# cielavenir/7bgzf

Measured on NVIDIA B200. Metric: BGZF compress GB/s (uncompressed), higher is better.
Workload: dtype u8

## Files before the change

7bgzf_b200/csrc/bgzf_block.h:

```cpp
#ifndef BGZF_BLOCK_H
#define BGZF_BLOCK_H

#include <stdint.h>
#include <stdio.h>

#if defined(__CUDACC__)
#define BG_HD __host__ __device__ __forceinline__
#else
#define BG_HD static inline
#endif
#if defined(BG_CHECK) && defined(__CUDA_ARCH__)
#define BG_ASSERT(cond) do { if (!(cond)) { printf("BG_ASSERT failed: %s (%s:%d) block %d thread %d\n", #cond, __FILE__, __LINE__, (int)blockIdx.x, (int)threadIdx.x); __trap(); } } while (0)
#else
#define BG_ASSERT(cond) do { } while (0)
#endif


#define BG_MAX_BLOCK 65536u
#define BG_DATA_BYTES (BG_MAX_BLOCK + 32u)
#define BG_HASH_BITS 14
#define BG_HASH_SIZE (1u << BG_HASH_BITS)
#define BG_NOPOS 0xFFFFu
#define BG_CHUNK 68u
#define BG_THREADS 1024u
// ... 81 lines not shown
    const uint32_t *crcpow;
    const uint16_t *perm;
    uint32_t n;
    uint32_t frame;
    BgParams prm;
};

BG_HD uint32_t bg_frame(uint32_t hdr, uint32_t trl, uint32_t final, uint32_t piece, uint32_t hist = 0) { return hdr | (trl << 8) | (final << 16) | (piece << 17) | ((hist / BG_CHUNK) << 18); }
BG_HD uint32_t bg_f_hist(const BgCtx &c) { return (c.frame >> 18) * BG_CHUNK; }
BG_HD uint32_t bg_f_hdr(const BgCtx &c) { return c.frame & 0xffu; }
BG_HD uint32_t bg_f_trl(const BgCtx &c) { return (c.frame >> 8) & 0xffu; }
BG_HD uint32_t bg_f_final(const BgCtx &c) { return (c.frame >> 16) & 1u; }
BG_HD bool bg_f_piece(const BgCtx &c) { return (c.frame >> 17) & 1u; }


BG_HD uint32_t bg_ld32(const uint32_t *w, uint32_t p)
{
    uint32_t i = p >> 2, s = (p & 3u) * 8u;
    uint32_t lo = w[i], hi = w[i + 1];
#if defined(__CUDA_ARCH__)
    return __funnelshift_r(lo, hi, p << 3);
#else
    return s ? (lo >> s) | (hi << (32u - s)) : lo;
#endif
}

BG_HD uint32_t bg_ld8(const uint32_t *w, uint32_t p) { return ((const uint8_t *)w)[p]; }

BG_HD uint32_t bg_funnel(uint32_t lo, uint32_t hi, uint32_t s)
{
#if defined(__CUDA_ARCH__)
    return __funnelshift_r(lo, hi, s);
#else
    return s ? (lo >> s) | (hi << (32u - s)) : lo;
#endif
}

BG_HD int bg_bsr(uint32_t v)
{
#if defined(__CUDA_ARCH__)
    return 31 - __clz(v);
#else
    return 31 - __builtin_clz(v);
#endif
}

BG_HD int bg_ctz(uint32_t v)
{
#if defined(__CUDA_ARCH__)
    return __ffs(v) - 1;
#else
    return __builtin_ctz(v);
#endif
}

BG_HD uint32_t bg_brev(uint32_t v, int nbits)
{
#if defined(__CUDA_ARCH__)
    return __brev(v) >> (32 - nbits);
#else
    uint32_t r = 0;
    for (int i = 0; i < nbits; i++)
        r |= ((v >> i) & 1u) << (nbits - 1 - i);
    return r;
#endif
}

BG_HD void bg_add32(uint32_t *a, uint32_t v)
{
#if defined(__CUDA_ARCH__)
    atomicAdd(a, v);
#else
    *a += v;
#endif
}

BG_HD uint32_t bg_fetch_add32(uint32_t *a, uint32_t v)
{
#if defined(__CUDA_ARCH__)
    return atomicAdd(a, v);
#else
    uint32_t old = *a;
    *a += v;
    return old;
#endif
}

BG_HD void bg_or32(uint32_t *a, uint32_t v)
{
#if defined(__CUDA_ARCH__)
    atomicOr(a, v);
#else
    *a |= v;
#endif
}

BG_HD uint32_t bg_len_slot(uint32_t len, uint32_t *nextra, uint32_t *extra)
{
    uint32_t l = len - 3;
    if (l < 8) { *nextra = 0; *extra = 0; return l; }
    if (len == 258) { *nextra = 0; *extra = 0; return 28; }
    uint32_t nb = (uint32_t)bg_bsr(l) - 2;
    *nextra = nb;
    *extra = l & ((1u << nb) - 1);
    return 8 + 4 * (nb - 1) + ((l >> nb) & 3);
}

BG_HD uint32_t bg_off_slot(uint32_t off, uint32_t *nextra, uint32_t *extra)
{
    uint32_t d = off - 1;
    if (d < 4) { *nextra = 0; *extra = 0; return d; }
    uint32_t b = (uint32_t)bg_bsr(d);
    *nextra = b - 1;
    *extra = d & ((1u << (b - 1)) - 1);
    return 2 * b + ((d >> (b - 1)) & 1);
}

BG_HD uint32_t bg_len_slot_extra_bits(uint32_t slot) { return slot < 8 || slot == 28 ? 0 : (slot - 4) >> 2; }
BG_HD uint32_t bg_off_slot_extra_bits(uint32_t slot) { return slot < 4 ? 0 : (slot - 2) >> 1; }

BG_HD uint32_t bg_static_llen(uint32_t sym) { return sym < 144 ? 8 : sym < 256 ? 9 : sym < 280 ? 7 : 8; }


#define BG_CRC_POLY 0xEDB88320u

BG_HD uint32_t bg_crc_mul(uint32_t a, uint32_t b)
{
    uint32_t p = 0;
    for (int i = 0; i < 32; i++) {
        p ^= b & (0u - ((a >> (31 - i)) & 1u));
        b = (b >> 1) ^ (BG_CRC_POLY & (0u - (b & 1u)));
    }
    return p;
}

BG_HD uint32_t bg_crc_byte(const uint32_t *tab, uint32_t r, uint32_t b) { return tab[(r ^ b) & 0xff] ^ (r >> 8); }

BG_HD uint32_t bg_mw(uint32_t len, uint32_t off) { return (len << 16) | (0xffffu - off); }
BG_HD uint32_t bg_mw_off(uint32_t r) { return 0xffffu - (r & 0xffffu); }


BG_HD void bg_phase_init(const BgCtx &c, uint32_t t, uint32_t T)
{
    for (uint32_t i = t; i < BG_HASH_SIZE; i += T)
        c.head[i] = BG_NOPOS;
    if (t < 256)
        c.litflag[t] = 0;
    if (t < 28)
        ((uint8_t *)c.dataw)[c.n + t] = 0;
    if (t < BG_S_COUNT)
        c.scal[t] = 0;
}

BG_HD void bg_phase_scan(const BgCtx &c, uint32_t t, uint32_t T)
{
    const uint32_t n = c.n;
    for (uint32_t p = t; p < n; p += T)
        c.litflag[bg_ld8(c.dataw, p)] = 1;
    const uint32_t hw = bg_f_hist(c) >> 2;
    const uint32_t m = (n >> 2) - hw;
    const uint32_t k = T - 1 - t;
    const uint32_t endw = m >= BG_CRC_WORDS * k ? m - BG_CRC_WORDS * k : 0;
    const uint32_t begw = endw >= BG_CRC_WORDS ? endw - BG_CRC_WORDS : 0;
    uint32_t r = 0;
    if (endw > begw) {
        r = begw == 0 ? 0xFFFFFFFFu : 0u;
        for (uint32_t w = begw; w < endw; w++) {
            uint32_t v = c.dataw[hw + w];
            r = bg_crc_byte(c.crctab, r, v & 0xff);
            r = bg_crc_byte(c.crctab, r, (v >> 8) & 0xff);
            r = bg_crc_byte(c.crctab, r, (v >> 16) & 0xff);
            r = bg_crc_byte(c.crctab, r, v >> 24);
        }
        r = bg_crc_mul(r, c.crcpow[k]);
    }
#if defined(__CUDA_ARCH__)
    for (int d = 16; d > 0; d >>= 1)
        r ^= __shfl_xor_sync(0xffffffffu, r, d);
    if ((t & 31u) == 0 && r)
        atomicXor(&c.scal[BG_S_CRC], r);
#else
    c.scal[BG_S_CRC] ^= r;
#endif
}

BG_HD void bg_phase_count(const BgCtx &c, uint32_t t, uint32_t T)
{
    (void)T;
    if (t < 256 && c.litflag[t])
        bg_add32(&c.scal[BG_S_NUSED], 1);
}

BG_HD uint32_t bg_min_match_len(uint32_t nused, int depth, uint32_t n)
{
    uint32_t ml;
    if (n < 512) return 3;
    ml = nused < 6 ? 9 : nused < 8 ? 8 : nused < 10 ? 7 : nused < 16 ? 6 : nused < 45 ? 5 : nused < 80 ? 4 : 3;
    if (depth < 16) {
        uint32_t cap = depth < 5 ? 4 : depth < 10 ? 5 : 7;
        if (ml > cap) ml = cap;
    }
    return ml;
}

BG_HD void bg_phase_settle(const BgCtx &c, uint32_t t, uint32_t T)
{
    (void)T;
    if (t != 0) return;
    const uint32_t n = c.n;
    uint32_t r = c.scal[BG_S_CRC];
    if (((n - bg_f_hist(c)) >> 2) == 0) r = 0xFFFFFFFFu;
    for (uint32_t p = n & ~3u; p < n; p++)
        r = bg_crc_byte(c.crctab, r, bg_ld8(c.dataw, p));
    c.scal[BG_S_CRC] = ~r;
    c.scal[BG_S_MINLEN] = bg_min_match_len(c.scal[BG_S_NUSED], c.prm.depth, n);
    c.scal[BG_S_DEPTH] = c.scal[BG_S_NUSED] >= 80 && c.prm.opt_passes == 0 ? (uint32_t)c.prm.depth + ((uint32_t)c.prm.depth + 1) / 2 : (uint32_t)c.prm.depth;
    c.scal[BG_S_HBYTES] = bg_min_match_len(c.scal[BG_S_NUSED], 1000, n) >= 5 ? (uint32_t)c.prm.hlong : 4u;
    if (c.scal[BG_S_MINLEN] == 3 && c.prm.depth >= 8) c.scal[BG_S_HBYTES] = 3;
}

BG_HD uint32_t bg_hash(const uint32_t *dataw, uint32_t p, uint32_t hbytes)
{
    uint32_t v = bg_ld32(dataw, p);
    if (hbytes == 3) v &= 0xffffffu;
    uint32_t h = v * 0x1E35A7BDu;
    if (hbytes == 5)
        h ^= bg_ld8(dataw, p + 4) * 0x9E3779B1u;
    else if (hbytes == 8)
        h ^= bg_ld32(dataw, p + 4) * 0x9E3779B1u;
    return h >> (32 - BG_HASH_BITS);
}

BG_HD void bg_phase_hash(const BgCtx &c, uint32_t t, uint32_t T)
{
    const uint32_t n = c.n, hb = c.scal[BG_S_HBYTES];
    for (uint32_t p = t; p < n; p += T)
        c.prev[p] = (p + hb <= n) ? (uint16_t)bg_hash(c.dataw, p, hb) : (uint16_t)BG_NOPOS;
}

BG_HD void bg_build_sequential(const BgCtx &c)
{
    for (uint32_t p = 0; p < c.n; p++) {
        uint32_t h = c.prev[p];
        if (h == BG_NOPOS) continue;
        c.prev[p] = c.head[h];
        c.head[h] = (uint16_t)p;
    }
}

BG_HD uint32_t bg_match_len(const uint32_t *dw, uint32_t p, uint32_t q, uint32_t l, uint32_t maxl)
{
    if (l >= maxl) return maxl;
    const uint32_t sp = (p & 3u) * 8u, sq = (q & 3u) * 8u;
    const uint32_t *wp = dw + ((p + l) >> 2), *wq = dw + ((q + l) >> 2);
    uint32_t plo = wp[0], qlo = wq[0];
    for (;;) {
        const uint32_t p1 = wp[1], q1 = wq[1], p2 = wp[2], q2 = wq[2];
        const uint32_t x1 = bg_funnel(plo, p1, sp) ^ bg_funnel(qlo, q1, sq);
        if (x1) { l += (uint32_t)bg_ctz(x1) >> 3; break; }
        const uint32_t x2 = bg_funnel(p1, p2, sp) ^ bg_funnel(q1, q2, sq);
        if (x2) { l += 4u + ((uint32_t)bg_ctz(x2) >> 3); break; }
        l += 8;
        if (l >= maxl) break;
        plo = p2;
        qlo = q2;
        wp += 2;
        wq += 2;
    }
    return l > maxl ? maxl : l;
}

BG_HD bool bg_in_window(uint32_t p, uint32_t q) { return p - q - 1u < 32768u; }


#define BG_B_TODO 0u
#define BG_B_MARK 8192u
#define BG_B_QUEUE 8192u
#define BG_B_RINGR 20480u
#define BG_B_RING 28672u
#define BG_QUEUE_WORDS 96u
#define BG_SCAN_CHUNK 2u
#define BG_QUEUE_WORDS_SHALLOW 160u
#define BG_SCAN_CHUNK_SHALLOW 4u

BG_HD bool bg_match_ok(uint32_t r, uint32_t minlen);

struct BgSearchPrm {
    uint32_t depth, nice, minlen;
    bool h3;
};
BG_HD BgSearchPrm bg_search_prm(const BgCtx &c)
{
    BgSearchPrm s;
    s.depth = c.scal[BG_S_DEPTH];
    s.nice = (uint32_t)c.prm.nice;
    s.minlen = c.scal[BG_S_MINLEN];
    s.h3 = c.scal[BG_S_HBYTES] == 3;
    return s;
}

template <bool H3>
BG_HD uint32_t bg_nearest_t(const BgCtx &c, const BgSearchPrm &sp, uint32_t p, bool *deep, uint32_t *target)
{
    uint32_t maxl = c.n - p;
    if (maxl > 258) maxl = 258;
    *deep = false;
    *target = p + 1;
    if (maxl < (uint32_t)BG_MIN_LOOKUP) return 0;
    const uint32_t q = c.prev[p];
    if (!bg_in_window(p, q)) return 0;
    const uint32_t *dw = c.dataw;
    uint32_t len = 3;
    if (H3) {
        len = 2;
        if (((bg_ld32(dw, q) ^ bg_ld32(dw, p)) & 0xffffffu) == 0) len = bg_match_len(dw, p, q, 0, maxl);
    } else if (bg_ld32(dw, q) == bg_ld32(dw, p)) {
        len = bg_match_len(dw, p, q, 4, maxl);
    }
    *deep = sp.depth > 1 && len < sp.nice && len < maxl && bg_in_window(p, c.prev[q]);
    if (len <= (H3 ? 2u : 3u)) return 0;
    const uint32_t r = bg_mw(len, p - q);
    if (bg_match_ok(r, sp.minlen)) *target = p + len;
    return r;
}
BG_HD uint32_t bg_nearest(const BgCtx &c, const BgSearchPrm &sp, uint32_t p, bool *deep, uint32_t *target)
{
    return sp.h3 ? bg_nearest_t<true>(c, sp, p, deep, target) : bg_nearest_t<false>(c, sp, p, deep, target);
}

BG_HD uint32_t bg_off_bin(uint32_t off) { return off <= 32u ? 0u : off <= 512u ? 1u : off <= 8192u ? 2u : 3u; }

BG_HD void bg_cand_init(const BgCtx &c, uint32_t p, uint32_t r)
{
    uint32_t *cd = c.cand + 4u * p;
    const uint32_t k = r ? bg_off_bin(bg_mw_off(r)) : 4u;
    cd[0] = k == 0 ? r : 0u; cd[1] = k == 1 ? r : 0u; cd[2] = k == 2 ? r : 0u; cd[3] = k == 3 ? r : 0u;
}

BG_HD void bg_phase_search_clear(const BgCtx &c, uint32_t t, uint32_t T)
{
    uint32_t *w = (uint32_t *)(c.regb + BG_B_TODO);
    for (uint32_t i = t; i < (BG_B_MARK + 8256u) / 4u; i += T) w[i] = 0;
}

BG_HD void bg_phase_search1(const BgCtx &c, uint32_t t, uint32_t T)
{
    uint32_t *elig = (uint32_t *)(c.regb + BG_B_TODO), *mark = (uint32_t *)(c.regb + BG_B_MARK);
    const uint32_t hist = bg_f_hist(c);
    if (t == 0) bg_or32(&mark[hist >> 5], 1u << (hist & 31u));
    const BgSearchPrm sp = bg_search_prm(c);
    for (uint32_t p = t; p < c.n; p += T) {
        bool deep;
        uint32_t target;
        if (p < hist) {
            c.R[p] = 0;
            if (c.prm.opt_passes > 0) bg_cand_init(c, p, 0);
            continue;
        }
        c.R[p] = bg_nearest(c, sp, p, &deep, &target);
        if (c.prm.opt_passes > 0) bg_cand_init(c, p, c.R[p]);
        if (deep) bg_or32(&elig[p >> 5], 1u << (p & 31u));
        bg_or32(&mark[target >> 5], 1u << (target & 31u));
    }
}

BG_HD void bg_phase_search_todo(const BgCtx &c, uint32_t t, uint32_t T, uint32_t own, uint32_t parts)
{
    uint32_t *todo = (uint32_t *)(c.regb + BG_B_TODO);
    const uint32_t *mark = (const uint32_t *)(c.regb + BG_B_MARK);
    for (uint32_t i = t; i < 2048u; i += T) {
        const uint32_t m = mark[i], pm = i ? mark[i - 1] : 0u;
// ... 1192 lines not shown
```

7bgzf_b200/csrc/bgzf_compress.cu:

```cuda
#include <cuda_runtime.h>
#include <stdint.h>

#include <atomic>
#include <cstring>

#include "bgzf_block.h"
#include "bgzf_kernels.h"

#define SM_DATA 0u
#define SM_REGA (BG_DATA_BYTES)
#define SM_REGB (SM_REGA + 131072u)
#define SM_CRCTAB (SM_REGB + 32768u)
#define SM_LITFLAG (SM_CRCTAB + 1024u)
#define SM_SCAL (SM_LITFLAG + 256u)
#define SM_MBAR (SM_SCAL + 4u * BG_S_COUNT)
#define SM_FRONTIER (SM_MBAR + 8u)
#define SM_SCAN (SM_MBAR + 16u)
#define SM_READY (SM_SCAN + 4u * 36u)
#define SM_TOTAL (SM_READY + 128u)

extern "C" size_t bgzf_compress_smem_bytes(void) { return SM_TOTAL; }

__device__ __forceinline__ uint32_t smem_u32(const void *p) { return (uint32_t)__cvta_generic_to_shared(p); }

// ... 460 lines not shown
            }
        }
    }
    __syncwarp();
    drain_queue<H3>(c, queue, 0u, cnt, lane);
}

__device__ __forceinline__ uint32_t cluster_rank()
{
    uint32_t r;
    asm volatile("mov.u32 %0, %%cluster_ctarank;" : "=r"(r));
    return r;
}
__device__ __forceinline__ uint32_t cluster_size()
{
    uint32_t r;
    asm volatile("mov.u32 %0, %%cluster_nctarank;" : "=r"(r));
    return r;
}
__device__ __forceinline__ void cluster_sync()
{
    asm volatile("barrier.cluster.arrive.release.aligned;\n\tbarrier.cluster.wait.acquire.aligned;" ::: "memory");
}

__device__ __forceinline__ void dp_segment_warp(const BgCtx &c, uint32_t w, uint32_t lane, uint32_t *ring)
{
    uint32_t a, b, e;
    bg_dp_segment_bounds(c.n, w, 32, &a, &b, &e);
    if (a >= b) return;
    const uint8_t *rb = c.regb;
    const uint4 *cand4 = (const uint4 *)c.cand;
    uint4 *stage = (uint4 *)(c.regb + BG_B_XTAB) + w * 32u;
    if (lane == 0) ring[e & (BG_DP_RING - 1)] = 0;
    const uint4 zero4 = make_uint4(0, 0, 0, 0);
    uint32_t top = e - 1;
    uint4 next = top >= lane && top - lane >= a ? __ldcg(cand4 + (top - lane)) : zero4;
    for (;;) {
        const uint4 mine = next;
        const uint32_t q = top - lane;
        const bool more = top >= a + 32u;
        if (more) next = top - 32u >= lane && top - 32u - lane >= a ? __ldcg(cand4 + (top - 32u - lane)) : zero4;
        {
            uint32_t oc = 0, litc = 0, m0 = 0, m1 = 0, m2 = 0, m3 = 0;
            if (top >= lane && q >= a) {
                const uint32_t cd[4] = { mine.x, mine.y, mine.z, mine.w };
#pragma unroll
                for (int k = 0; k < 4; k++) {
                    uint32_t nbx, exx;
                    if (cd[k]) oc |= (uint32_t)rb[BG_B_OFFCOST + bg_off_slot(bg_mw_off(cd[k]), &nbx, &exx)] << (8 * k);
                }
                m0 = mine.x >> 16;
                m1 = max(m0, mine.y >> 16);
                m2 = max(m1, mine.z >> 16);
                m3 = max(m2, mine.w >> 16);
                litc = rb[BG_B_LITCOST + bg_ld8(c.dataw, q)];
            }
            stage[lane] = make_uint4(m0 | (m1 << 16), m2 | (m3 << 16), oc, litc);
        }
        __syncwarp();
        const uint32_t steps = top - a + 1 < 32u ? top - a + 1 : 32u;
        uint32_t mybest = 0;
        for (uint32_t j = 0; j < steps; j++) {
            const uint32_t p = top - j;
            const uint4 st = stage[j];
            const uint32_t M0 = st.x & 0xffffu, M1 = st.x >> 16, M2 = st.y & 0xffffu, M3 = st.y >> 16;
            uint32_t maxl = e - p;
            if (M3 < maxl) maxl = M3;
            uint32_t best = 0xffffffffu;
            if (lane == 0) best = bg_dp_pack(st.w + ring[(p + 1) & (BG_DP_RING - 1)], 1, 0);
            uint32_t l = 3 + lane;
            if (l <= maxl) {
#pragma unroll 1
                do {
                    const uint32_t k = (l > M0 ? 1u : 0u) + (l > M1 ? 1u : 0u) + (l > M2 ? 1u : 0u);
                    const uint32_t oc = (st.z >> (8 * k)) & 0xffu;
                    const uint32_t v = bg_dp_pack(rb[BG_B_LENCOST + l] + oc + ring[(p + l) & (BG_DP_RING - 1)], l, k);
                    best = v < best ? v : best;
                    l += 32;
                } while (l <= maxl);
            }
            best = __reduce_min_sync(0xffffffffu, best);
            if (lane == j) {
                ring[p & (BG_DP_RING - 1)] = best >> 11;
                mybest = best;
            }
            __syncwarp();
        }
        if (lane < steps && q < b) {
            const uint32_t l = (mybest >> 2) & 511u, k = mybest & 3u;
            if (l == 1) {
                c.stepcode[q] = 0;
            } else {
                const uint32_t off = bg_mw_off(k == 0 ? mine.x : k == 1 ? mine.y : k == 2 ? mine.z : mine.w);
                c.stepcode[q] = (uint8_t)(l <= 256 ? l - 2 : 255);
                c.R[q] = bg_mw(l, off);
            }
        }
        if (!more) break;
        top -= 32u;
    }
}

__device__ __forceinline__ uint32_t chunk_class(const BgCtx &c, uint32_t ch)
{
    if (ch * BG_CHUNK >= c.n) return 0u;
    const uint32_t *sc = (const uint32_t *)(c.stepcode + ch * BG_CHUNK);
    uint32_t zeros = 0;
#pragma unroll
    for (uint32_t k = 0; k < BG_CHUNK / 4u; k++) {
        const uint32_t v = sc[k];
        zeros += __popc((v - 0x01010101u) & ~v & 0x80808080u);
    }
    return zeros >= 64u ? 7u : zeros >> 3;
}

__device__ __forceinline__ void chunk_order_count(const BgCtx &c, uint32_t t, uint32_t &cls, uint32_t &rank)
{
    const uint32_t lane = t & 31u, warp = t >> 5;
    uint32_t *cnt = (uint32_t *)(c.regb + BG_B_CLASSCNT);
    cls = chunk_class(c, t);
    rank = 0;
#pragma unroll
    for (uint32_t k = 0; k < 8u; k++) {
        const unsigned m = __ballot_sync(0xffffffffu, cls == k);
        if (cls == k) rank = __popc(m & ((1u << lane) - 1u));
        if (lane == k) cnt[k * 32u + warp] = __popc(m);
    }
}

__device__ __forceinline__ void chunk_order_scan(const BgCtx &c, uint32_t t)
{
    if (t >= 32u) return;
    uint32_t *cnt = (uint32_t *)(c.regb + BG_B_CLASSCNT);
    uint32_t v[8], sum = 0;
#pragma unroll
    for (uint32_t k = 0; k < 8u; k++) { v[k] = cnt[t * 8u + k]; sum += v[k]; }
    uint32_t inc = sum;
    for (int d = 1; d < 32; d <<= 1) {
        const uint32_t y = __shfl_up_sync(0xffffffffu, inc, d);
        if (t >= (uint32_t)d) inc += y;
    }
    uint32_t run = inc - sum;
#pragma unroll
    for (uint32_t k = 0; k < 8u; k++) { cnt[t * 8u + k] = run; run += v[k]; }
}

__device__ __forceinline__ void chunk_order_place(const BgCtx &c, uint32_t t, uint32_t cls, uint32_t rank)
{
    const uint32_t *cnt = (const uint32_t *)(c.regb + BG_B_CLASSCNT);
    BG_ASSERT(cls < 8u && cnt[cls * 32u + (t >> 5)] + rank < BG_MAX_CHUNKS);
    ((uint16_t *)(c.regb + BG_B_PERM))[cnt[cls * 32u + (t >> 5)] + rank] = (uint16_t)t;
}

__device__ __forceinline__ void bitonic_sort_512(uint32_t *keys, uint32_t t)
{
    for (uint32_t k = 2; k <= 512; k <<= 1) {
        for (uint32_t j = k >> 1; j > 0; j >>= 1) {
            if (t < 512) {
                uint32_t x = t ^ j;
                if (x > t) {
                    uint32_t a = keys[t], b = keys[x];
                    bool up = (t & k) == 0;
                    if ((a > b) == up) { keys[t] = b; keys[x] = a; }
                }
            }
            __syncthreads();
        }
    }
}

__device__ __forceinline__ uint32_t block_exclusive_scan_1024(uint32_t *v, uint32_t *scratch, uint32_t t)
{
    const uint32_t lane = t & 31u, warp = t >> 5;
    uint32_t x = v[t], inc = x;
    for (int d = 1; d < 32; d <<= 1) {
        uint32_t y = __shfl_up_sync(0xffffffffu, inc, d);
        if (lane >= (uint32_t)d) inc += y;
    }
    if (lane == 31) scratch[warp] = inc;
    __syncthreads();
    if (warp == 0) {
        uint32_t w = scratch[lane], winc = w;
        for (int d = 1; d < 32; d <<= 1) {
            uint32_t y = __shfl_up_sync(0xffffffffu, winc, d);
            if (lane >= (uint32_t)d) winc += y;
        }
        scratch[lane] = winc - w;
        if (lane == 31) scratch[32] = winc;
    }
    __syncthreads();
    v[t] = scratch[warp] + inc - x;
    uint32_t total = scratch[32];
    __syncthreads();
    return total;
}

__device__ __forceinline__ void gather_member(const uint32_t *src, uint32_t n, uint8_t *dst, uint32_t t, uint32_t nthr)
{
    const uint32_t head = (uint32_t)((4u - ((uintptr_t)dst & 3u)) & 3u);
    if (n <= head + 4) {
        for (uint32_t i = t; i < n; i += nthr) dst[i] = (uint8_t)(__ldcg(src + (i >> 2)) >> (8u * (i & 3u)));
        return;
    }
    if (t < head) dst[t] = (uint8_t)(__ldcg(src) >> (8u * t));
    const uint32_t words = (n - head) >> 2;
    uint32_t *dw = (uint32_t *)(dst + head);
    const uint32_t sh = head * 8u;
    for (uint32_t i = t; i < words; i += nthr)
        dw[i] = __funnelshift_r(__ldcg(src + i), __ldcg(src + i + 1), sh);
    const uint32_t done = head + words * 4u;
    if (t < n - done) dst[done + t] = (uint8_t)(__ldcg(src + ((done + t) >> 2)) >> (8u * ((done + t) & 3u)));
}

__device__ __forceinline__ uint32_t block_exclusive_scan_1024(uint32_t *v, uint32_t *scratch, uint32_t t);

__device__ __forceinline__ void fused_compaction(const BgzfCompressArgs &a, uint32_t *v, uint32_t *scratch, uint32_t t)
{
    uint64_t carry = *a.gather_total;
    for (uint32_t start = 0; start < a.nblocks; start += 1024u) {
        const uint32_t i = start + t;
        v[t] = i < a.nblocks ? __ldcg(a.out_len + i) : 0u;
        __syncthreads();
        const uint32_t total = block_exclusive_scan_1024(v, scratch, t);
        if (i < a.nblocks) a.gather_off[i] = carry + v[t];
        carry += total;
        __syncthreads();
    }
    if (t == 0) *a.gather_total = carry;
    __syncthreads();
    const uint32_t grp = t >> 8, gt = t & 255u;
    for (uint32_t b = grp; b < a.nblocks; b += BG_THREADS / 256u) {
        BG_ASSERT(__ldcg(a.out_len + b) <= BG_SLOT_BYTES && a.gather_off[b] + __ldcg(a.out_len + b) <= carry);
        gather_member((const uint32_t *)(a.slots + (size_t)b * BG_SLOT_BYTES), __ldcg(a.out_len + b), a.gather_out + a.gather_off[b], gt, 256u);
    }
}

#define PROF_MARK(i)                                                        \
    do {                                                                    \
        if (prof && t == 0) {                                               \
            long long now_ = clock64();                                     \
            atomicAdd((unsigned long long *)&prof[i], (unsigned long long)(now_ - tprev_)); \
            tprev_ = now_;                                                  \
        }                                                                   \
    } while (0)

template <bool SPLIT>
__device__ __forceinline__ void compress_blocks(BgzfCompressArgs &a)
{
    extern __shared__ __align__(128) uint8_t smem[];
    const uint32_t t = threadIdx.x, T = BG_THREADS;
    uint64_t *mbar = (uint64_t *)(smem + SM_MBAR);
    uint32_t *scan_scratch = (uint32_t *)(smem + SM_SCAN);
    unsigned long long *prof = a.prof;
    long long tprev_ = prof ? clock64() : 0;
    uint32_t *const pscr = scan_scratch;

    BgCtx c;
    c.dataw = (uint32_t *)(smem + SM_DATA);
    c.prev = (uint16_t *)(smem + SM_REGA);
    c.stepcode = smem + SM_REGA;
    c.jump8 = smem + SM_REGA + 65536u;
    c.offarr = (uint16_t *)(smem + SM_REGA + 65536u);
    c.head = (uint16_t *)(smem + SM_REGB);
    c.regb = smem + SM_REGB;
    c.crctab = (uint32_t *)(smem + SM_CRCTAB);
    c.litflag = smem + SM_LITFLAG;
    c.scal = (uint32_t *)(smem + SM_SCAL);
    const uint32_t crank = SPLIT ? cluster_rank() : 0u, csize = SPLIT ? cluster_size() : 1u;
    const uint32_t unit = SPLIT ? blockIdx.x / csize : blockIdx.x;
    uint32_t *const unit_scratch = a.scratch + (size_t)unit * (SPLIT ? BGZF_SCRATCH_WORDS + BGZF_SPLIT_EXTRA_WORDS : BGZF_SCRATCH_WORDS);
    c.R = unit_scratch;
    c.cand = a.cand ? a.cand + (size_t)unit * (4u * BG_MAX_BLOCK) : nullptr;
    c.crcpow = a.crcpow;
    c.prm = a.prm;
    c.frame = bg_frame(a.hdr_bytes ? a.hdr_bytes : 18u, 8u, 1u, 0u);
    c.perm = (const uint16_t *)(smem + SM_REGB + BG_B_PERM);

    if (t < 256) c.crctab[t] = a.crctab[t];
    if (t == 0) {
        mbar_init(mbar, 1);
        asm volatile("fence.mbarrier_init.release.cluster;" ::: "memory");
    }
    __syncthreads();
    uint32_t parity = 0;

    for (uint32_t b = unit; b < a.nblocks; b += SPLIT ? a.nblocks : gridDim.x) {
        const uint8_t *src;
        uint32_t n;
        if (a.in_off) {
            src = a.in + a.in_off[b];
            n = a.in_len[b];
        } else {
            const uint64_t off = (uint64_t)b * a.block_size;
            src = a.in + off;
            const uint64_t rem = a.in_bytes - off;
            n = rem < a.block_size ? (uint32_t)rem : a.block_size;
        }
        c.out = (uint32_t *)(a.slots + (size_t)b * BG_SLOT_BYTES);
        if (a.piece_mode) {
            const uint64_t gb = a.piece_base + b;
            const bool first = gb % a.member_blocks == 0, last = (gb + 1) % a.member_blocks == 0 || gb + 1 == a.piece_total;
            uint32_t hist = 0;
            if (a.history && !first && !a.in_off) {
                const uint64_t in_member = (gb % a.member_blocks) * a.block_size, in_buffer = (uint64_t)a.lead + (uint64_t)b * a.block_size;
                uint64_t h = in_member < in_buffer ? in_member : in_buffer;
                if (h > a.history) h = a.history;
                hist = (uint32_t)h - (uint32_t)h % BG_HISTORY_STEP;
            }
            src -= hist;
            n += hist;
            c.frame = bg_frame(first ? a.head_gap : 0u, last ? a.tail_gap : 0u, last && !a.no_final ? 1u : 0u, 1u, hist);
        }
        c.n = n;

        const bool aligned = (((uintptr_t)src) & 15u) == 0;
        const uint32_t bulk = aligned ? (n & ~15u) : 0u;
        if (bulk) {
            if (t == 0) {
                fence_proxy_async();
                mbar_expect_tx(mbar, bulk);
                tma_load_1d(smem + SM_DATA, src, bulk, mbar);
            }
        }
        for (uint32_t i = bulk + t; i < n; i += T)
            smem[SM_DATA + i] = src[i];
        bg_phase_init(c, t, T);
        if (bulk) {
            mbar_wait(mbar, parity);
            parity ^= 1u;
        }
        __syncthreads();
        PROF_MARK(0);

        bg_phase_scan(c, t, T);
        __syncthreads();
        bg_phase_count(c, t, T);
        __syncthreads();
        bg_phase_settle(c, t, T);
        __syncthreads();
        PROF_MARK(1);
        PROF_MARK(2);
        uint4 *hi = (uint4 *)(c.R + BG_MAX_BLOCK + 32);
        if (SPLIT) {
            uint4 *xprev = (uint4 *)(unit_scratch + BGZF_SCRATCH_WORDS);
            build_peers_phase(c, hi, t & 31u, t >> 5, BG_THREADS / 32u, crank, csize, xprev, nullptr, nullptr, 0);
            cluster_sync();
            import_peer_tiles(c, xprev, t, crank, csize);
            __syncthreads();
            PROF_MARK(3);
            if (t < 32u * BG_LINKERS) build_link_phase(c, hi, t >> 5, t & 31u, &c.scal[BG_S_WLIST], nullptr, nullptr, 0);
        } else {
            volatile uint8_t *ready = (volatile uint8_t *)(smem + SM_READY);
            if (t < 128u) ready[t] = 0;
            if (prof && t == 0) { pscr[0] = 0; pscr[1] = 0; pscr[2] = 0xffffffffu; }
            __syncthreads();
            const long long t0 = prof ? clock64() : 0;
            if (t < 32u * BG_LINKERS) {
                build_link_phase(c, hi, t >> 5, t & 31u, &c.scal[BG_S_WLIST], ready, prof, t0);
            } else {
                build_peers_phase(c, hi, t & 31u, (t >> 5) - BG_LINKERS, BG_THREADS / 32u - BG_LINKERS, 0u, 1u, nullptr, ready, prof, t0);
                if (prof && (t & 31u) == 0) atomicMax(&pscr[0], (uint32_t)(clock64() - t0));
            }
        }
        __syncthreads();
        PROF_MARK(10);
        {
            bg_phase_search_clear(c, t, T);
            if (SPLIT) cluster_sync();
            else __syncthreads();
            const long long t1 = prof ? clock64() : 0;
            search_nearest<SPLIT>(c, t, crank, csize);
            if (!SPLIT && prof && (t & 31u) == 0) {
                const uint32_t d = (uint32_t)(clock64() - t1);
                atomicMax(&pscr[1], d);
                atomicMin(&pscr[2], d);
            }
            if (SPLIT) cluster_sync();
            else __syncthreads();
            if (!SPLIT && prof && t == 0) {
                atomicAdd(&prof[22], (unsigned long long)pscr[0]);
                atomicAdd(&prof[26], (unsigned long long)pscr[1]);
                atomicAdd(&prof[27], (unsigned long long)pscr[2]);
            }
            PROF_MARK(21);
            if (c.scal[BG_S_DEPTH] > 1) {
                bg_phase_search_todo(c, t, T, crank, csize);
                __syncthreads();
                const bool h3 = c.scal[BG_S_HBYTES] == 3;
                if (c.scal[BG_S_DEPTH] <= 24u) {
                    if (h3) search_deep_batches<true>(c, t, crank, csize);
                    else search_deep_batches<false>(c, t, crank, csize);
                } else {
                    if (h3) search_deep<true>(c, t, crank, csize);
                    else search_deep<false>(c, t, crank, csize);
                }
            }
        }
        if (SPLIT) {
            cluster_sync();
            if (crank) return;
        }
        __syncthreads();
        PROF_MARK(4);
        for (int pass = 0; pass <= c.prm.opt_passes; pass++) {
            if (pass == 0) {
                bg_phase_accept(c, t, T);
            } else {
                bg_phase_costs(c, t, T);
                __syncthreads();
                dp_segment_warp(c, t >> 5, t & 31u, (uint32_t *)(smem + SM_REGA + 65536u) + (t >> 5) * BG_DP_RING);
            }
            __syncthreads();
            if (bg_f_hist(c)) {
                bg_phase_history_steps(c, t, T);
                __syncthreads();
            }
            PROF_MARK(15);
            bg_phase_jump(c, t, T);
            __syncthreads();
            PROF_MARK(5);
            bg_phase_walk_clear(c, t, T);
            bg_phase_clear_freq(c, t, T);
            __syncthreads();
            bg_phase_walk_mark(c, t, T);
            __syncthreads();
            bg_phase_walk_list(c, t, T);
            __syncthreads();
            PROF_MARK(16);
            bg_phase_walk_a(c, t, T);
            __syncthreads();
            PROF_MARK(17);
            bg_phase_walk_b(c, t, T);
            uint32_t ccls, crnk;
            chunk_order_count(c, t, ccls, crnk);
            __syncthreads();
            PROF_MARK(18);
            bg_phase_walk_c(c, t, T);
            chunk_order_scan(c, t);
            __syncthreads();
            chunk_order_place(c, t, ccls, crnk);
            __syncthreads();
            PROF_MARK(6);
            bg_phase_tally(c, t, T);
            __syncthreads();
            bg_phase_lkeys(c, t, T);
            __syncthreads();
            PROF_MARK(7);
            bitonic_sort_512((uint32_t *)(c.regb + BG_B_KEYS), t);
            PROF_MARK(11);
            bg_phase_huff_prep(c, t, T);
            __syncthreads();
            bg_phase_huff(c, t, T);
            __syncthreads();
            bg_phase_huff_depth(c, t, T);
            __syncthreads();
            bg_phase_huff_fix(c, t, T);
            __syncthreads();
            bg_phase_huff_assign(c, t, T);
            __syncthreads();
            PROF_MARK(12);
        }
        bg_phase_hdr1(c, t, T);
        __syncthreads();
        bg_phase_hdr2(c, t, T);
        __syncthreads();
        bg_phase_hdr3(c, t, T);
        __syncthreads();
        const uint32_t nitems = block_exclusive_scan_1024((uint32_t *)(c.regb + BG_B_CBITS), scan_scratch, t);
        bg_phase_hdr4(c, t, T);
        __syncthreads();
        bg_phase_hdr4b(c, t, T);
        __syncthreads();
        bg_phase_hdr5(c, t, T, nitems);
        __syncthreads();
        PROF_MARK(13);
        bg_phase_decide_b(c, t, T);
        __syncthreads();
        bg_phase_codes_a(c, t, T);
        __syncthreads();
        bg_phase_codes_b(c, t, T);
        __syncthreads();
        bg_phase_codes_c(c, t, T);
        __syncthreads();
        bg_phase_tabs(c, t, T);
        __syncthreads();
        PROF_MARK(8);
        bg_phase_hdr_bits(c, t, T);
        bg_phase_sizes(c, t, T);
        __syncthreads();
        PROF_MARK(19);
        block_exclusive_scan_1024((uint32_t *)(c.regb + BG_B_CBITS), scan_scratch, t);
        block_exclusive_scan_1024((uint32_t *)(c.regb + BG_B_IOFF), scan_scratch, t);
        PROF_MARK(20);
        bg_phase_zero_out(c, t, T);
        __syncthreads();
        PROF_MARK(14);
        bg_phase_emit(c, t, T);
        if (t == 0) {
            const uint32_t st = c.scal[BG_S_STATUS];
            a.out_len[b] = st ? 0u : bg_f_hdr(c) + c.scal[BG_S_PAYLOAD] + bg_f_trl(c);
            if (a.crc_out) a.crc_out[b] = c.scal[BG_S_CRC];
            a.status[b] = st;
            if (st) atomicOr(a.err_flag, 1u);
        }
        fence_proxy_async();
        __syncthreads();
        PROF_MARK(9);
    }
    if (!SPLIT && a.gather_out) {
        __threadfence();
        __syncthreads();
        if (t == 0) scan_scratch[35] = atomicAdd(a.done_count, 1u) == gridDim.x - 1u ? 1u : 0u;
        __syncthreads();
        if (scan_scratch[35]) {
            __threadfence();
            fused_compaction(a, (uint32_t *)(smem + SM_REGB), scan_scratch, t);
        }
    }
}

__global__ void __launch_bounds__(BG_THREADS, 1)
bgzf_compress_kernel(BgzfCompressArgs a)
{
    compress_blocks<false>(a);
}

__global__ void __launch_bounds__(BG_THREADS, 1)
bgzf_compress_split_kernel(BgzfCompressArgs a)
{
    compress_blocks<true>(a);
}

__global__ void __launch_bounds__(1024, 1)
bgzf_scan_kernel(const uint32_t *len, uint64_t *off, uint32_t nmax, const uint64_t *count_dev, const uint64_t *base_dev,
                 uint64_t *total_out)
{
    __shared__ uint32_t v[1024];
    __shared__ uint32_t scratch[36];
    const uint32_t t = threadIdx.x;
    uint32_t n = nmax;
    if (count_dev) { const uint64_t cd = *count_dev; n = cd < nmax ? (uint32_t)cd : nmax; }
    uint64_t carry = base_dev ? *base_dev : 0ull;
    __syncthreads();
    for (uint32_t start = 0; start < n; start += 1024) {
        const uint32_t i = start + t;
        v[t] = i < n ? len[i] : 0u;
        __syncthreads();
        const uint32_t total = block_exclusive_scan_1024(v, scratch, t);
        if (i < n) off[i] = carry + v[t];
        carry += total;
        __syncthreads();
    }
    if (t == 0) *total_out = carry;
}

__global__ void __launch_bounds__(256)
bgzf_gather_kernel(const uint8_t *slots, const uint32_t *len, const uint64_t *off, uint32_t nblocks, uint8_t *out,
                   const uint64_t *total, int append_eof)
{
    const uint32_t b = blockIdx.x, t = threadIdx.x;
    if (b == nblocks) {
        if (append_eof && t < 28) {
            const uint8_t eof[28] = { 0x1f, 0x8b, 0x08, 0x04, 0, 0, 0, 0, 0, 0xff, 0x06, 0, 0x42, 0x43, 0x02, 0,
                                      0x1b, 0, 0x03, 0, 0, 0, 0, 0, 0, 0, 0, 0 };
            out[*total + t] = eof[t];
        }
        return;
    }
    const uint32_t n = len[b];
    const uint32_t *src = (const uint32_t *)(slots + (size_t)b * BG_SLOT_BYTES);
    uint8_t *dst = out + off[b];
    const uint32_t head = (uint32_t)((4u - ((uintptr_t)dst & 3u)) & 3u);
    if (n <= head + 4) {
        for (uint32_t i = t; i < n; i += blockDim.x) dst[i] = ((const uint8_t *)src)[i];
        return;
    }
    if (t < head) dst[t] = ((const uint8_t *)src)[t];
    const uint32_t words = (n - head) >> 2;
    uint32_t *dw = (uint32_t *)(dst + head);
    const uint32_t sh = head * 8u;
    for (uint32_t i = t; i < words; i += blockDim.x)
        dw[i] = __funnelshift_r(src[i], src[i + 1], sh);
    const uint32_t done = head + words * 4u;
    if (t < n - done) dst[done + t] = ((const uint8_t *)src)[done + t];
}

__global__ void __launch_bounds__(256)
bgzf_deliver_kernel(const uint8_t *slots, const uint32_t *len, const uint64_t *out_off, uint8_t *host_out, uint32_t n)
{
    const uint32_t b = blockIdx.x, t = threadIdx.x;
    if (b >= n) return;
    const uint32_t nbytes = len[b];
    const uint4 *src = (const uint4 *)(slots + (size_t)b * BG_SLOT_BYTES);
    uint4 *dst = (uint4 *)(host_out + out_off[b]);
    for (uint32_t i = t; i < (nbytes + 15u) / 16u; i += blockDim.x) dst[1u + i] = src[i];
    if (t == 0) dst[0] = make_uint4(nbytes, 0u, 0u, 0u);
}

extern "C" cudaError_t bgzf_launch_deliver(const uint8_t *slots, const uint32_t *len, const uint64_t *out_off, uint8_t *host_out, uint32_t n,
                                           cudaStream_t stream)
{
    bgzf_deliver_kernel<<<n, 256, 0, stream>>>(slots, len, out_off, host_out, n);
    return cudaGetLastError();
}

extern "C" cudaError_t bgzf_launch_compress(const BgzfCompressArgs *a, int grid, cudaStream_t stream)
{
    static std::atomic<unsigned long long> configured{0};
    int dev = 0;
    cudaGetDevice(&dev);
    if (!((configured.load() >> dev) & 1ull)) {
        cudaError_t e = cudaFuncSetAttribute(bgzf_compress_kernel, cudaFuncAttributeMaxDynamicSharedMemorySize, (int)SM_TOTAL);
        if (e != cudaSuccess) return e;
        configured.fetch_or(1ull << dev);
    }
    bgzf_compress_kernel<<<grid, BG_THREADS, SM_TOTAL, stream>>>(*a);
    return cudaGetLastError();
}

extern "C" cudaError_t bgzf_launch_compress_split(const BgzfCompressArgs *a, int csize, cudaStream_t stream)
{
    static std::atomic<unsigned long long> configured{0};
    int dev = 0;
    cudaGetDevice(&dev);
    if (!((configured.load() >> dev) & 1ull)) {
        cudaError_t e = cudaFuncSetAttribute(bgzf_compress_split_kernel, cudaFuncAttributeMaxDynamicSharedMemorySize, (int)SM_TOTAL);
// ... 35 lines not shown
```

Measured before the change: 32.99.

## Overlap CRC with Huffman tree build and replace bitonic sort with rank sort

Splits the CRC computation out of the initial scan so that it runs on the idle warps while four warps build the Huffman trees behind a named barrier. The 512-element bitonic sort, with its many block-wide barriers, is replaced by a direct counting rank for the literal/length keys. Distance-tree construction and the precode header are done by single warps. The aim is to cut block-wide synchronisation and serial phases in the per-block pipeline. The cost is more complex warp specialisation, and the CRC now depends on a pass==0 condition in the non-split path.

```diff
diff --git a/7bgzf_b200/csrc/bgzf_block.h b/7bgzf_b200/csrc/bgzf_block.h
--- a/7bgzf_b200/csrc/bgzf_block.h
+++ b/7bgzf_b200/csrc/bgzf_block.h
@@ -257,36 +257,58 @@
         c.scal[t] = 0;
 }
 
+BG_HD void bg_phase_census(const BgCtx &c, uint32_t t, uint32_t T)
+{
+    for (uint32_t p = t; p < c.n; p += T)
+        c.litflag[bg_ld8(c.dataw, p)] = 1;
+}
+
+BG_HD void bg_crc_slices(const BgCtx &c, uint32_t u, uint32_t U)
+{
+    const uint32_t hw = bg_f_hist(c) >> 2;
+    const uint32_t m = (c.n >> 2) - hw;
+    const uint32_t *d = c.dataw + hw;
+    uint32_t acc = 0;
+    for (uint32_t k0 = u; k0 < BG_THREADS; k0 += 2 * U) {
+        const uint32_t k1 = k0 + U;
+        const uint32_t e0 = m >= BG_CRC_WORDS * k0 ? m - BG_CRC_WORDS * k0 : 0;
+        const uint32_t e1 = k1 < BG_THREADS && m >= BG_CRC_WORDS * k1 ? m - BG_CRC_WORDS * k1 : 0;
+        const uint32_t b0 = e0 >= BG_CRC_WORDS ? e0 - BG_CRC_WORDS : 0, b1 = e1 >= BG_CRC_WORDS ? e1 - BG_CRC_WORDS : 0;
+        if (e0 == b0) break;
+        uint32_t r0 = b0 == 0 ? 0xFFFFFFFFu : 0u, r1 = b1 == 0 ? 0xFFFFFFFFu : 0u;
+        for (uint32_t i = 0; i < BG_CRC_WORDS; i++) {
+            if (b0 + i < e0) {
+                const uint32_t v = d[b0 + i];
+                r0 = bg_crc_byte(c.crctab, r0, v & 0xff);
+                r0 = bg_crc_byte(c.crctab, r0, (v >> 8) & 0xff);
+                r0 = bg_crc_byte(c.crctab, r0, (v >> 16) & 0xff);
+                r0 = bg_crc_byte(c.crctab, r0, v >> 24);
+            }
+            if (b1 + i < e1) {
+                const uint32_t v = d[b1 + i];
+                r1 = bg_crc_byte(c.crctab, r1, v & 0xff);
+                r1 = bg_crc_byte(c.crctab, r1, (v >> 8) & 0xff);
+                r1 = bg_crc_byte(c.crctab, r1, (v >> 16) & 0xff);
+                r1 = bg_crc_byte(c.crctab, r1, v >> 24);
+            }
+        }
+        acc ^= bg_crc_mul(r0, c.crcpow[k0]);
+        if (e1 > b1) acc ^= bg_crc_mul(r1, c.crcpow[k1]);
+    }
+#if defined(__CUDA_ARCH__)
+    for (int s = 16; s > 0; s >>= 1)
+        acc ^= __shfl_xor_sync(0xffffffffu, acc, s);
+    if ((u & 31u) == 0 && acc)
+        atomicXor(&c.scal[BG_S_CRC], acc);
+#else
+    c.scal[BG_S_CRC] ^= acc;
+#endif
+}
+
 BG_HD void bg_phase_scan(const BgCtx &c, uint32_t t, uint32_t T)
 {
-    const uint32_t n = c.n;
-    for (uint32_t p = t; p < n; p += T)
-        c.litflag[bg_ld8(c.dataw, p)] = 1;
-    const uint32_t hw = bg_f_hist(c) >> 2;
-    const uint32_t m = (n >> 2) - hw;
-    const uint32_t k = T - 1 - t;
-    const uint32_t endw = m >= BG_CRC_WORDS * k ? m - BG_CRC_WORDS * k : 0;
-    const uint32_t begw = endw >= BG_CRC_WORDS ? endw - BG_CRC_WORDS : 0;
-    uint32_t r = 0;
-    if (endw > begw) {
-        r = begw == 0 ? 0xFFFFFFFFu : 0u;
-        for (uint32_t w = begw; w < endw; w++) {
-            uint32_t v = c.dataw[hw + w];
-            r = bg_crc_byte(c.crctab, r, v & 0xff);
-            r = bg_crc_byte(c.crctab, r, (v >> 8) & 0xff);
-            r = bg_crc_byte(c.crctab, r, (v >> 16) & 0xff);
-            r = bg_crc_byte(c.crctab, r, v >> 24);
-        }
-        r = bg_crc_mul(r, c.crcpow[k]);
-    }
-#if defined(__CUDA_ARCH__)
-    for (int d = 16; d > 0; d >>= 1)
-        r ^= __shfl_xor_sync(0xffffffffu, r, d);
-    if ((t & 31u) == 0 && r)
-        atomicXor(&c.scal[BG_S_CRC], r);
-#else
-    c.scal[BG_S_CRC] ^= r;
-#endif
+    bg_phase_census(c, t, T);
+    bg_crc_slices(c, t, T);
 }
 
 BG_HD void bg_phase_count(const BgCtx &c, uint32_t t, uint32_t T)
@@ -308,20 +330,31 @@
     return ml;
 }
 
-BG_HD void bg_phase_settle(const BgCtx &c, uint32_t t, uint32_t T)
-{
-    (void)T;
-    if (t != 0) return;
+BG_HD void bg_crc_finish(const BgCtx &c)
+{
     const uint32_t n = c.n;
     uint32_t r = c.scal[BG_S_CRC];
     if (((n - bg_f_hist(c)) >> 2) == 0) r = 0xFFFFFFFFu;
     for (uint32_t p = n & ~3u; p < n; p++)
         r = bg_crc_byte(c.crctab, r, bg_ld8(c.dataw, p));
     c.scal[BG_S_CRC] = ~r;
+}
+
+BG_HD void bg_phase_settle_census(const BgCtx &c, uint32_t t, uint32_t T)
+{
+    (void)T;
+    if (t != 0) return;
+    const uint32_t n = c.n;
     c.scal[BG_S_MINLEN] = bg_min_match_len(c.scal[BG_S_NUSED], c.prm.depth, n);
     c.scal[BG_S_DEPTH] = c.scal[BG_S_NUSED] >= 80 && c.prm.opt_passes == 0 ? (uint32_t)c.prm.depth + ((uint32_t)c.prm.depth + 1) / 2 : (uint32_t)c.prm.depth;
     c.scal[BG_S_HBYTES] = bg_min_match_len(c.scal[BG_S_NUSED], 1000, n) >= 5 ? (uint32_t)c.prm.hlong : 4u;
     if (c.scal[BG_S_MINLEN] == 3 && c.prm.depth >= 8) c.scal[BG_S_HBYTES] = 3;
+}
+
+BG_HD void bg_phase_settle(const BgCtx &c, uint32_t t, uint32_t T)
+{
+    if (t == 0) bg_crc_finish(c);
+    bg_phase_settle_census(c, t, T);
 }
 
 BG_HD uint32_t bg_hash(const uint32_t *dataw, uint32_t p, uint32_t hbytes)
diff --git a/7bgzf_b200/csrc/bgzf_compress.cu b/7bgzf_b200/csrc/bgzf_compress.cu
--- a/7bgzf_b200/csrc/bgzf_compress.cu
+++ b/7bgzf_b200/csrc/bgzf_compress.cu
@@ -636,21 +636,123 @@
     ((uint16_t *)(c.regb + BG_B_PERM))[cnt[cls * 32u + (t >> 5)] + rank] = (uint16_t)t;
 }
 
-__device__ __forceinline__ void bitonic_sort_512(uint32_t *keys, uint32_t t)
-{
-    for (uint32_t k = 2; k <= 512; k <<= 1) {
-        for (uint32_t j = k >> 1; j > 0; j >>= 1) {
-            if (t < 512) {
-                uint32_t x = t ^ j;
-                if (x > t) {
-                    uint32_t a = keys[t], b = keys[x];
-                    bool up = (t & k) == 0;
-                    if ((a > b) == up) { keys[t] = b; keys[x] = a; }
-                }
-            }
-            __syncthreads();
-        }
-    }
+#define BG_B_RANKKEYS BG_B_TREEP
+
+__device__ __forceinline__ void litlen_keys(const BgCtx &c, uint32_t t)
+{
+    const uint32_t *lfreq = (const uint32_t *)(c.regb + BG_B_LFREQ);
+    if (t < 288) {
+        const uint32_t f = lfreq[t];
+        ((uint32_t *)(c.regb + BG_B_RANKKEYS))[t] = f ? (f << 9) | t : 0xFFFFFFFFu;
+        if (f) atomicAdd(&c.scal[BG_S_HM], 1u);
+    }
+}
+
+__device__ __forceinline__ void litlen_rank(const BgCtx &c, uint32_t t)
+{
+    uint8_t *rb = c.regb;
+    if (t < 288) {
+        const uint4 *all = (const uint4 *)(rb + BG_B_RANKKEYS);
+        const uint32_t k = ((const uint32_t *)all)[t];
+        rb[BG_B_LLEN + t] = 0;
+        if (k != 0xFFFFFFFFu) {
+            uint32_t rank = 0;
+#pragma unroll 8
+            for (uint32_t j = 0; j < 72; j++) {
+                const uint4 q = all[j];
+                rank += (q.x < k) + (q.y < k) + (q.z < k) + (q.w < k);
+            }
+            ((uint32_t *)(rb + BG_B_KEYS))[rank] = k;
+            ((uint32_t *)(rb + BG_B_TREEW))[rank] = k >> 9;
+        }
+    } else if (t < 288 + 30) {
+        if (bg_rank_key((const uint32_t *)(rb + BG_B_DFREQ), 30, t - 288, (uint32_t *)(rb + BG_B_DKEYS))) atomicAdd(&c.scal[BG_S_DM], 1u);
+    } else if (t < 288 + 32 + 16) {
+        ((uint32_t *)(rb + BG_B_BLC))[t - 320] = 0;
+        if (t == 320) c.scal[BG_S_HOVF] = 0;
+    }
+}
+
+__device__ __forceinline__ void warp_huff_lengths(const uint32_t *keys, uint32_t m, uint32_t maxbits, uint32_t nzero, uint32_t *w,
+                                                  uint16_t *par, uint32_t *blc, uint8_t *lens, uint32_t lane)
+{
+    if (lane < nzero) lens[lane] = 0;
+    if (lane < m) w[lane] = keys[lane] >> 9;
+    if (lane < 16) blc[lane] = 0;
+    __syncwarp();
+    if (m < 2) {
+        if (lane == 0) {
+            const uint32_t s = m ? keys[0] & 511u : 0u;
+            lens[s] = 1;
+            lens[s ? 0 : 1] = 1;
+        }
+        return;
+    }
+    if (lane == 0) bg_huff_merge(m, w, par);
+    __syncwarp();
+    const uint32_t root = 2 * m - 2;
+    uint32_t ovf = 0;
+    for (uint32_t i = lane; i < root; i += 32) {
+        uint32_t d = 0;
+        for (uint32_t x = i; x != root && d < 64; x = par[x]) d++;
+        if (d > maxbits) { d = maxbits; ovf++; }
+        if (i < m) atomicAdd(&blc[d], 1u);
+    }
+    int overflow = (int)__reduce_add_sync(0xffffffffu, ovf);
+    __syncwarp();
+    if (lane == 0) {
+        while (overflow > 0) {
+            uint32_t bits = maxbits - 1;
+            while (bits > 1 && blc[bits] == 0) bits--;
+            blc[bits]--;
+            blc[bits + 1] += 2;
+            blc[maxbits]--;
+            overflow -= 2;
+        }
+    }
+    __syncwarp();
+    for (uint32_t i = lane; i < m; i += 32) {
+        uint32_t bits = maxbits, cum = blc[maxbits];
+        while (cum <= i && bits > 1) cum += blc[--bits];
+        lens[keys[i] & 511u] = (uint8_t)bits;
+    }
+}
+
+__device__ __forceinline__ void dist_tree_warp(const BgCtx &c, uint32_t lane)
+{
+    uint8_t *rb = c.regb;
+    warp_huff_lengths((const uint32_t *)(rb + BG_B_DKEYS), c.scal[BG_S_DM], 15, 32, (uint32_t *)(rb + BG_B_DTREEW),
+                      (uint16_t *)(rb + BG_B_DTREEP), (uint32_t *)(rb + BG_B_SCRATCH) + 32, rb + BG_B_DLEN, lane);
+}
+
+__device__ __forceinline__ void precode_hdr_warp(const BgCtx &c, uint32_t lane, uint32_t nitems)
+{
+    uint8_t *rb = c.regb;
+    uint32_t nl, nd;
+    bg_hdr_dims(c, &nl, &nd);
+    const uint32_t *pfreq = (const uint32_t *)(rb + BG_B_PFREQ);
+    uint8_t *plen = rb + BG_B_PLEN;
+    warp_huff_lengths((const uint32_t *)(rb + BG_B_PKEYS), c.scal[BG_S_PM], 7, 19, (uint32_t *)(rb + BG_B_DTREEW),
+                      (uint16_t *)(rb + BG_B_DTREEP), (uint32_t *)(rb + BG_B_SCRATCH) + 16, plen, lane);
+    __syncwarp();
+    const unsigned used = __ballot_sync(0xffffffffu, lane < 19 && plen[bg_precode_order(lane)] != 0);
+    uint32_t np = used ? 32u - (uint32_t)__clz(used) : 0u;
+    if (np < 4) np = 4;
+    const uint32_t bits = lane < 19 ? pfreq[lane] * (plen[lane] + (lane == 16 ? 2u : lane == 17 ? 3u : lane == 18 ? 7u : 0u)) : 0u;
+    const uint32_t hdr = 3 + 5 + 5 + 4 + 3 * np + __reduce_add_sync(0xffffffffu, bits);
+    if (lane == 0) {
+        c.scal[BG_S_DYNHDR] = hdr;
+        c.scal[BG_S_NITEMS] = nitems;
+        c.scal[BG_S_NL] = nl;
+        c.scal[BG_S_ND] = nd;
+        c.scal[BG_S_NP] = np;
+    }
+}
+
+#define BG_TREE_WARPS 4u
+__device__ __forceinline__ void tree_bar()
+{
+    asm volatile("bar.sync 1, %0;" :: "n"(BG_TREE_WARPS * 32) : "memory");
 }
 
 __device__ __forceinline__ uint32_t block_exclusive_scan_1024(uint32_t *v, uint32_t *scratch, uint32_t t)
@@ -816,11 +918,11 @@
         __syncthreads();
         PROF_MARK(0);
 
-        bg_phase_scan(c, t, T);
+        bg_phase_census(c, t, T);
         __syncthreads();
         bg_phase_count(c, t, T);
         __syncthreads();
-        bg_phase_settle(c, t, T);
+        bg_phase_settle_census(c, t, T);
         __syncthreads();
         PROF_MARK(1);
         PROF_MARK(2);
@@ -927,23 +1029,34 @@
             PROF_MARK(6);
             bg_phase_tally(c, t, T);
             __syncthreads();
-            bg_phase_lkeys(c, t, T);
-            __syncthreads();
             PROF_MARK(7);
-            bitonic_sort_512((uint32_t *)(c.regb + BG_B_KEYS), t);
+            litlen_keys(c, t);
+            if (prof && t == 0) { pscr[3] = 0; pscr[4] = 0; }
+            __syncthreads();
+            litlen_rank(c, t);
+            __syncthreads();
             PROF_MARK(11);
-            bg_phase_huff_prep(c, t, T);
-            __syncthreads();
-            bg_phase_huff(c, t, T);
-            __syncthreads();
-            bg_phase_huff_depth(c, t, T);
-            __syncthreads();
-            bg_phase_huff_fix(c, t, T);
-            __syncthreads();
-            bg_phase_huff_assign(c, t, T);
-            __syncthreads();
+            const long long t2 = prof ? clock64() : 0;
+            if (t < 32u * BG_TREE_WARPS) {
+                const uint32_t TT = 32u * BG_TREE_WARPS;
+                if (t < 32u) bg_phase_huff(c, t, TT);
+                else if (t < 64u) dist_tree_warp(c, t - 32u);
+                tree_bar();
+                bg_phase_huff_depth(c, t, TT);
+                tree_bar();
+                bg_phase_huff_fix(c, t, TT);
+                tree_bar();
+                bg_phase_huff_assign(c, t, TT);
+                if (prof && pass == 0 && (t & 31u) == 0) atomicMax(&pscr[3], (uint32_t)(clock64() - t2));
+            } else if (pass == 0) {
+                bg_crc_slices(c, t - 32u * BG_TREE_WARPS, T - 32u * BG_TREE_WARPS);
+                if (prof && (t & 31u) == 0) atomicMax(&pscr[4], (uint32_t)(clock64() - t2));
+            }
+            __syncthreads();
+            if (prof && pass == 0 && t == 0 && pscr[4] > pscr[3]) atomicAdd(&prof[28], (unsigned long long)(pscr[4] - pscr[3]));
             PROF_MARK(12);
         }
+        if (t == 0) bg_crc_finish(c);
         bg_phase_hdr1(c, t, T);
         __syncthreads();
         bg_phase_hdr2(c, t, T);
@@ -953,9 +1066,11 @@
         const uint32_t nitems = block_exclusive_scan_1024((uint32_t *)(c.regb + BG_B_CBITS), scan_scratch, t);
         bg_phase_hdr4(c, t, T);
         __syncthreads();
-        bg_phase_hdr4b(c, t, T);
-        __syncthreads();
-        bg_phase_hdr5(c, t, T, nitems);
+        if (t < 32u) {
+            bg_phase_hdr4b(c, t, 32u);
+            __syncwarp();
+            precode_hdr_warp(c, t, nitems);
+        }
         __syncthreads();
         PROF_MARK(13);
         bg_phase_decide_b(c, t, T);
```

Result: faster. 34.20 (median of 6 runs) (+3.7%).
